# CycloneBoy/pdf_table

Measured on AMD Instinct MI355X. Metric: pages/s, higher is better.
Workload: dtype bf16

## Files before the change

### pdf_table_amd/csrc/c_api.hip

```cpp
#include <stdarg.h>
#include <stdio.h>
#include <stdlib.h>

#include <cmath>

#include "common.h"

namespace PT_FMT_NS {
namespace api {

static int ensure(void** buf, size_t* cap, size_t need);

int pt_engine_check(pt_engine* e) {
  PT_REQUIRE(e, "pt_engine_check: null engine");
  if (e->lstm_err && *e->lstm_err) {
    *e->lstm_err = 0;
    e->lstm_cluster = 0;
    pt_set_error("lstm_cluster_kernel: a workgroup waited > 2^22 polls for its peers -- the launch was not co-resident "
                 "(GPU shared with another process or stream?).  The recognition results since the last check are invalid; "
                 "this engine now uses the streaming LSTM kernel (pt_engine_set_lstm_cluster(e, 0)): run the batch again");
    return PT_ERR_HIP;
  }
  return PT_OK;
}
// ... 430 lines not shown
  return PT_OK;
}

int pt_det_box_scores(pt_engine* e, const float* d_prob, int n, int net_h, int net_w, const float* d_boxes, int nb,
                      float* d_scores, pt_stream stream) {
  PT_REQUIRE(e && d_prob && (nb == 0 || (d_boxes && d_scores)), "pt_det_box_scores: bad arguments");
  return pt_launch_box_scores(d_prob, n, net_h, net_w, d_boxes, nb, d_scores, reinterpret_cast<hipStream_t>(stream));
}

static int ensure(void** buf, size_t* cap, size_t need) {
  if (need <= *cap) return PT_OK;
  PT_HIP_CHECK(hipDeviceSynchronize());
  if (*buf) PT_HIP_CHECK(hipFree(*buf));
  *buf = nullptr;
  *cap = 0;
  PT_HIP_CHECK(hipMalloc(buf, need));
  *cap = need;
  return PT_OK;
}

static int rec_microbatch() {
  static int mb = -1;
  if (mb < 0) {
    const char* s = getenv("PT_REC_MICROBATCH");
    mb = s ? atoi(s) : 6144;
    if (mb < 1) mb = 1;
  }
  return mb;
}

static int rec_pre_chunk(pt_engine* e, const uint8_t* d_pages, int n_pages, int h, int w, const pt_rec_line* d_lines,
                         const int64_t* h_crop_px, int i0, int nb, bf16_t* d_gray, hipStream_t s) {
  (void)n_pages;
  long long maxpx = 0, total = 0;
  for (int i = 0; i < nb; ++i) {
    const long long px = h_crop_px[i0 + i] > 0 ? h_crop_px[i0 + i] : 0;
    total += px;
    if (px > maxpx) maxpx = px;
  }
  int rc;
  if ((rc = ensure(&e->rec_off, &e->rec_off_cap, (size_t)(nb + 1) * sizeof(long long))) != PT_OK) return rc;
  if ((rc = ensure(&e->rec_crops, &e->rec_crops_cap, (size_t)total * 3 + 16)) != PT_OK) return rc;
  if ((rc = pt_launch_rec_offsets(d_lines + i0, nb, reinterpret_cast<long long*>(e->rec_off), s)) != PT_OK) return rc;
  const long long* d_off = reinterpret_cast<const long long*>(e->rec_off);
  {
    PtProfScope ps(e, s, PT_PROF_OTHER, 0, "rec warp");
    rc = pt_launch_rec_warp(d_pages, h, w, d_lines + i0, nb, d_off, reinterpret_cast<uint8_t*>(e->rec_crops), (int)maxpx, s);
    if (rc != PT_OK) return rc;
  }
  PtProfScope ps(e, s, PT_PROF_OTHER, 0, "rec resize+gray");
  return pt_launch_rec_resize_gray(reinterpret_cast<const uint8_t*>(e->rec_crops), d_lines + i0, d_off, nb,
                                   pt_split(e), d_gray, s);
}

int pt_rec_preprocess(pt_engine* e, const uint8_t* d_pages_rgb, int n_pages, int h, int w, const pt_rec_line* d_lines,
                      const int64_t* h_crop_px, int n_lines, uint16_t* d_gray, pt_stream stream) {
  PT_REQUIRE(e && d_pages_rgb && d_lines && h_crop_px && d_gray && n_lines > 0, "pt_rec_preprocess: bad arguments");
  PT_HIP_CHECK(hipSetDevice(e->device));
  return rec_pre_chunk(e, d_pages_rgb, n_pages, h, w, d_lines, h_crop_px, 0, n_lines, d_gray, reinterpret_cast<hipStream_t>(stream));
}

static int upload_crop_offsets(pt_engine* e, const std::vector<long long>& off, hipStream_t s) {
  const size_t nb = off.size() * sizeof(long long);
  void* hs = e->stage_ring.acquire(nb);
  PT_REQUIRE(hs, "recognition: pinned staging (%s)", hipGetErrorString(hipGetLastError()));
  memcpy(hs, off.data(), nb);
// ... 546 lines not shown
```

### pdf_table_amd/csrc/common.h

```cpp
#pragma once
#include <hip/hip_runtime.h>
#include <stdint.h>
#include <string.h>

#include <map>
#include <string>
#include <vector>

#include "../../include/pdftable_hip.h"
#include "act16.h"

typedef uint16_t bf16_t;

void pt_set_error(const char* fmt, ...);

#define PT_HIP_CHECK(expr)                                                                  \
  do {                                                                                      \
    hipError_t _e = (expr);                                                                 \
    if (_e != hipSuccess) {                                                                 \
      pt_set_error("%s failed: %s (%s:%d)", #expr, hipGetErrorString(_e), __FILE__, __LINE__); \
      return PT_ERR_HIP;                                                                    \
    }                                                                                       \
  } while (0)

// ... 240 lines not shown
                            float* logits, int split, hipStream_t s);
int pt_launch_db_head_mfma(const bf16_t* in, int B, int H, int W, const bf16_t* w3, const float* b3, const bf16_t* w6,
                           const float* b6, float* prob, float* logits, hipStream_t s, uint32_t* bitmap = nullptr, float thresh = 0.f);
int pt_launch_bitmap(const float* prob, int n, int H, int W, float thresh, int dilate, uint32_t* bitmap,
                     hipStream_t s);
int pt_launch_box_scores(const float* prob, int n, int H, int W, const float* boxes, int nb, float* scores,
                         hipStream_t s);

#define PT_SE_CHUNKS 64
int pt_launch_stem3x3s2(const bf16_t* in, const float* w, const float* b, bf16_t* out, int B, int H, int W, int split,
                        hipStream_t s, int variant);
int pt_launch_dwconv(const bf16_t* in, const float* w, const float* b, bf16_t* out, int B, int H, int W, int C, int k,
                     int stride, int act, int split, hipStream_t s, const float* slope);
int pt_launch_se(const bf16_t* x, const float* w1, const float* b1, const float* w2, const float* b2, float* gate,
                 bf16_t* out, int B, int HW, int C, int split, hipStream_t s, int hidden, int mode, float* part);
int pt_launch_add(const bf16_t* a, const bf16_t* b, bf16_t* out, long long npix, int C, int split, hipStream_t s);
int pt_launch_chan_mean(const bf16_t* x, int B, int HW, int C, int split, float* part, bf16_t* mean, int rows, hipStream_t s);
int pt_pplcnet_forward_net(pt_engine* e, int slot, const bf16_t* x, int n, int H, int W, int textline, float* logits,
                           int* n_classes, hipStream_t s, int arena);
int pt_launch_cls_resize_norm(const uint8_t* base, const pt_cls_image* images, int n, int max_h, int max_w, int OH, int OW,
                              const float* lut, int split, bf16_t* out, hipStream_t s);
int pt_launch_cls_desc_from_lines(const pt_rec_line* lines, const long long* off, int n, pt_cls_image* images, hipStream_t s);
int pt_launch_cls_line_resize_norm(const uint8_t* pages, int ph, int pw, const pt_rec_line* lines, int n, int max_h, int max_w, int OH,
                                   int OW, const float* lut, int split, bf16_t* out, hipStream_t s);
int pt_launch_dbnas_tail(const bf16_t* y, const float* tw, int B, int H4, int W4, int split, float* prob, float* logits,
                         hipStream_t s);
int pt_dbnas_forward_net(pt_engine* e, const bf16_t* x, int n, int H, int W, float* prob, float* logits, hipStream_t s);

int pt_launch_rec_offsets(const pt_rec_line* lines, int n, long long* off, hipStream_t s);
int pt_launch_rec_warp(const uint8_t* pages, int ph, int pw, const pt_rec_line* lines, int n_lines,
                       const long long* pix_off, uint8_t* crops, int max_crop_px, hipStream_t s);
int pt_launch_rec_resize_gray(const uint8_t* crops, const pt_rec_line* lines, const long long* pix_off, int n_lines,
                              int split, bf16_t* out, hipStream_t s);
int pt_launch_rec_pp_resize_norm(const uint8_t* crops, const pt_rec_line* lines, const long long* pix_off,
                                 const pt_rec_pp_item* items, int n_items, int img_h, int max_img_w, const float* lut, float* out,
                                 hipStream_t s);
struct PtCrnnLimits {
  int* lim[6];
  int* cols;
  int* glist;
  int* blist3a;
  int* blist2a;
  int* blist2b;
};
int pt_launch_rows_live_list(const int* lim, int n, int* glist, hipStream_t s);
int pt_launch_crnn_limits(const pt_rec_line* lines, int n, const PtCrnnLimits& L, hipStream_t s);
int pt_launch_crnn_fill(bf16_t* out, const bf16_t* ref, const int* lim, int tile_w, int div, int n, int rows, int W, int cs,
                        hipStream_t s, const int* end_lim = nullptr, int end_tile = 1);
int pt_launch_crnn_conv0_pool(const bf16_t* in, int n, int H, int W, const float* w64x9, const float* bias, int split,
                              bf16_t* out, hipStream_t s, const int* xlim = nullptr);
int pt_launch_maxpool_kxk(const bf16_t* in, int n, int H, int W, int C, int kh, int kw, int h2c, int split, bf16_t* out,
                          hipStream_t s);
int pt_launch_lstm(pt_engine* e, const bf16_t* gx, const bf16_t* whh, bf16_t* hout, int B, int T, int split, hipStream_t s);
int pt_launch_gemm_argmax(const bf16_t* A, long long M, int K, const bf16_t* W, const float* bias, int N, int* ids, float* maxv,
                          hipStream_t s);
int pt_launch_gemm_argmax_x3(const bf16_t* A, long long M, int K, const bf16_t* W3, const float* bias, int N, int n_real, int* ids, float* maxv,
                             void* scratch, hipStream_t s);
int pt_launch_gemm_rows_x3(const bf16_t* A, long long M, int K, const bf16_t* W3, const float* bias, int N, bf16_t* out, int relu, hipStream_t s,
                           const int* tlim = nullptr);
int pt_launch_gemm_rows(const bf16_t* A, long long M, int K, const bf16_t* W, const float* bias, int N, bf16_t* out, int relu,
                        hipStream_t s, const int* tlim = nullptr);
int pt_launch_argmax_reduce(const float* part, long long rows, int ntiles, int* ids, float* maxv, hipStream_t s);
int pt_crnn_forward_net(pt_engine* e, const bf16_t* gray, int n, int32_t* ids, float* maxlogit, hipStream_t s,
                        const pt_rec_line* d_lines = nullptr);

int pt_cvit_forward_net(pt_engine* e, const float* gray, int layout, int n, int32_t* ids, float* maxlogit, hipStream_t s,
// ... 89 lines not shown
```

### pdf_table_amd/csrc/det_kernels.hip

```cpp
#include <math.h>

#include "common.h"

namespace PT_FMT_NS {

typedef __attribute__((ext_vector_type(4))) uint32_t u32x4;
typedef __attribute__((ext_vector_type(2))) uint32_t u32x2;

__device__ __forceinline__ float bf2f(uint32_t bits16) { return a16_to_f32(bits16); }
__device__ __forceinline__ uint32_t f2bf(float f) { return f32_to_a16(f); }

struct ResizeCoef {
  int s0, s1;
  int a0, a1;
};
__device__ __forceinline__ ResizeCoef resize_coef(int d, double scale, int ssize, bool clamp_frac) {
  float f = (float)(((double)d + 0.5) * scale - 0.5);
  int s = (int)floorf(f);
  f -= (float)s;
  ResizeCoef c;
  if (clamp_frac) {
    if (s < 0) { f = 0.f; s = 0; }
    if (s >= ssize - 1) { f = 0.f; s = ssize - 1; }
  }
  c.a0 = (int)rintf((1.f - f) * 2048.f);
  c.a1 = (int)rintf(f * 2048.f);
  int t0 = s, t1 = s + 1;
  t0 = t0 < 0 ? 0 : (t0 >= ssize ? ssize - 1 : t0);
  t1 = t1 < 0 ? 0 : (t1 >= ssize ? ssize - 1 : t1);
  c.s0 = t0;
  c.s1 = t1;
  return c;
}

constexpr int PRE_ROWS = 8;

__global__ __launch_bounds__(256) void det_preprocess_kernel(const uint8_t* __restrict__ pages, int n, int h, int w,
                                                              int nh, int nw, int flavour, int split, bf16_t* __restrict__ out,
                                                              double sx, double sy) {
  a16_kernel_enter();
  __shared__ uint32_t lut[3][256];
  {
    const int u = threadIdx.x;
#pragma unroll
    for (int c = 0; c < 3; ++c) {
      float o;
      if (flavour == PT_DET_PRE_DB_TORCH) {
        const float mean[3] = {123.68f, 116.78f, 103.94f};
        o = ((float)u - mean[c]) / 255.f;
      } else {
        const float scale = (float)(1.0 / 255.0);
        const float mean[3] = {0.485f, 0.456f, 0.406f};
        const float stdv[3] = {0.229f, 0.224f, 0.225f};
        o = ((float)u * scale - mean[c]) / stdv[c];
      }
      const uint32_t hi = f2bf(o);
      lut[c][u] = hi | (f2bf(o - bf2f(hi)) << 16);
    }
  }
  __syncthreads();
  const bool area2 = (w == 2 * nw) && (h == 2 * nh);
  const int b = blockIdx.z;
  const uint8_t* src = pages + (size_t)b * h * w * 3;
  for (int x = blockIdx.x * blockDim.x + threadIdx.x; x < nw; x += gridDim.x * blockDim.x) {
    const ResizeCoef cx = resize_coef(x, sx, w, true);
    const int o0 = cx.s0 * 3, d1 = (cx.s1 - cx.s0) * 24;
    for (int ry = 0; ry < PRE_ROWS; ++ry) {
      const int y = blockIdx.y * PRE_ROWS + ry;
      if (y >= nh) break;
      const long long i = ((long long)b * nh + y) * nw + x;
      int v[3];
      if (w == nw && h == nh) {
        const uint8_t* p = src + ((size_t)y * w + x) * 3;
        v[0] = p[0]; v[1] = p[1]; v[2] = p[2];
      } else if (area2) {
        const uint8_t* p0 = src + ((size_t)(2 * y) * w + 2 * x) * 3;
        const uint8_t* p1 = p0 + (size_t)w * 3;
#pragma unroll
        for (int c = 0; c < 3; ++c) v[c] = (p0[c] + p0[3 + c] + p1[c] + p1[3 + c] + 2) >> 2;
      } else {
        const ResizeCoef cy = resize_coef(y, sy, h, false);
        const uint8_t* r0 = src + (size_t)cy.s0 * w * 3;
        const uint8_t* r1 = src + (size_t)cy.s1 * w * 3;
        unsigned long long q0, q1;
        if (o0 + 8 <= w * 3) {
          __builtin_memcpy(&q0, r0 + o0, 8);
          __builtin_memcpy(&q1, r1 + o0, 8);
        } else {
          q0 = q1 = 0;
          for (int k = 0; k < 3; ++k) {
            q0 |= (unsigned long long)r0[o0 + k] << (8 * k) | (unsigned long long)r0[cx.s1 * 3 + k] << (d1 + 8 * k);
            q1 |= (unsigned long long)r1[o0 + k] << (8 * k) | (unsigned long long)r1[cx.s1 * 3 + k] << (d1 + 8 * k);
          }
        }
#pragma unroll
        for (int c = 0; c < 3; ++c) {
          const int S0 = (int)((q0 >> (8 * c)) & 0xFF) * cx.a0 + (int)((q0 >> (d1 + 8 * c)) & 0xFF) * cx.a1;
          const int S1 = (int)((q1 >> (8 * c)) & 0xFF) * cx.a0 + (int)((q1 >> (d1 + 8 * c)) & 0xFF) * cx.a1;
          v[c] = (((cy.a0 * (S0 >> 4)) >> 16) + ((cy.a1 * (S1 >> 4)) >> 16) + 2) >> 2;
          v[c] = v[c] < 0 ? 0 : (v[c] > 255 ? 255 : v[c]);
        }
      }
      const uint32_t e0 = lut[0][v[2]], e1 = lut[1][v[1]], e2 = lut[2][v[0]];
      if (!split) {
        u32x2 pk;
        pk.x = (e0 & 0xFFFFu) | (e1 << 16);
        pk.y = e2 & 0xFFFFu;
        *reinterpret_cast<u32x2*>(out + (size_t)i * 4) = pk;
      } else {
        u32x4 pk;
        pk.x = (e0 & 0xFFFFu) | (e1 << 16);
        pk.y = e2 & 0xFFFFu;
        pk.z = (e0 >> 16) | (e1 & 0xFFFF0000u);
        pk.w = e2 >> 16;
        *reinterpret_cast<u32x4*>(out + (size_t)i * 8) = pk;
      }
    }
  }
}

int pt_launch_det_preprocess(const uint8_t* pages, int n, int h, int w, int nh, int nw, int flavour, int split,
                             bf16_t* out, hipStream_t s) {
  PT_REQUIRE(n > 0 && nh > 0 && nw > 0 && nh < 65536 && n < 65536, "det pre-process: bad extents %d x %d x %d", n, nh, nw);
  hipLaunchKernelGGL(det_preprocess_kernel, dim3((nw + 255) / 256, (nh + PRE_ROWS - 1) / PRE_ROWS, n), dim3(256), 0, s, pages, n, h, w, nh, nw, flavour, split, out,
                     (double)w / nw, (double)h / nh);
  PT_HIP_CHECK(hipGetLastError());
  return PT_OK;
}

__device__ __forceinline__ uint32_t bfmax2(uint32_t a, uint32_t b) {
  const float al = a16lo_f32(a), bl = a16lo_f32(b);
  const float ah = a16hi_f32(a), bh = a16hi_f32(b);
  const uint32_t lo = (bl > al) ? (b & 0xFFFFu) : (a & 0xFFFFu);
  const uint32_t hi = (bh > ah) ? (b & 0xFFFF0000u) : (a & 0xFFFF0000u);
  return lo | hi;
}

__global__ __launch_bounds__(256) void maxpool3x3s2_split_kernel(const bf16_t* __restrict__ in, int B, int H, int W,
                                                                  int C, bf16_t* __restrict__ out) {
  a16_kernel_enter();
  const int Ho = (H + 2 - 3) / 2 + 1, Wo = (W + 2 - 3) / 2 + 1;
  const int cg = C >> 3;
  const long long total = (long long)B * Ho * Wo * cg;
  for (long long i = (long long)blockIdx.x * blockDim.x + threadIdx.x; i < total; i += (long long)gridDim.x * blockDim.x) {
    const int g = (int)(i % cg);
    long long t = i / cg;
    const int ox = (int)(t % Wo);
    t /= Wo;
    const int oy = (int)(t % Ho);
    const int b = (int)(t / Ho);
    uint32_t bh[8], bl[8];
    float bv[8];
    bool first = true;
    for (int dy = 0; dy < 3; ++dy) {
      const int iy = oy * 2 - 1 + dy;
      if ((unsigned)iy >= (unsigned)H) continue;
      for (int dx = 0; dx < 3; ++dx) {
        const int ix = ox * 2 - 1 + dx;
// ... 483 lines not shown
```

### pdf_table_amd/csrc/dla_net.h

```cpp
#pragma once

#include <stdlib.h>

#include <string>
#include <vector>

#include "net_ctx.h"

namespace PT_FMT_NS {

int pt_launch_conv3x3_c16(pt_engine* e, const bf16_t* in, const bf16_t* w, const float* bias, bf16_t* out, int B, int H, int W,
                          int N, int stride, int split, hipStream_t s);
int pt_launch_dla_thin_chain(pt_engine* e, const bf16_t* in, int B, int H, int W, const bf16_t* w_stem, const float* b_stem, const bf16_t* w0,
                             const float* b0, const bf16_t* w1, const float* b1, bf16_t* out, hipStream_t s);

namespace {

struct DlaCtx : NetCtx {
  bf16_t* cols = nullptr;
  float* om = nullptr;
  const int* ylimit = nullptr;
  double alg_scale = 1.0;

  void conv(const T& in, const std::string& q, int N, int ks, int stride, const T& out, int relu, const T* res = nullptr,
            int nv = 0, float* out_f32 = nullptr, int f32_cs = 0, int cin_override = 0, int alg_n = 0) {
    ConvDesc c;
    if (!conv_desc(c, in, q, N, ks, stride, relu)) return;
    if (cin_override) c.Cin = cin_override;
    c.n_valid = nv; c.ylimit = ylimit; c.alg_n = alg_n; c.alg_scale = alg_scale;
    if (out_f32) to_f32(c, out_f32, f32_cs);
    else to_map(c, out);
    if (res) { c.res = res->p; c.res_mode = 1; }
    launch(c);
  }
  void conv_cat(const std::vector<T>& ins, const std::string& q, int N, const T& out, int relu) {
    const PtTensor* w = get(q + (x3 ? ".w3" : ".w"));
    const PtTensor* b = get(q + ".b");
    if (!go()) return;
    ConvDesc c;
    c.in = ins[0].p; c.B = n; c.H = ins[0].H; c.W = ins[0].W;
    c.nseg = (int)ins.size();
    c.Cin = 0;
    for (int i = 0; i < c.nseg; ++i) {
      c.seg_c[i] = ins[i].C;
      c.Cin += ins[i].C;
      if (i) c.in_more[i - 1] = ins[i].p;
    }
    c.w = W(w); c.bias = F(b);
    c.N = N; c.ks = 1; c.stride = 1; c.relu = relu; c.split = x3; c.alg_scale = alg_scale;
    to_map(c, out);
    launch(c);
  }
  T maxpool2(const T& x) {
    T o = alloc(x.H / 2, x.W / 2, x.C);
    if (go()) {
      e->prof.next_bytes = (double)n * x.H * x.W * x.C * 2.0 * mul * 1.25;
      PtProfScope ps(e, s, PT_PROF_OTHER, 0, "maxpool2x2");
      const int r = pt_launch_maxpool_kxk(x.p, n, x.H, x.W, x.C, 2, 2, 0, x3, o.p, s);
      if (r != PT_OK) rc = r;
    }
    return o;
  }
  T block(const std::string& q, const T& x, const T& residual, int stride, int cout) {
    T t = alloc(x.H / stride, x.W / stride, cout);
    conv(x, q + ".conv1", cout, 3, stride, t, 1);
    T o = alloc(t.H, t.W, cout);
    conv(t, q + ".conv2", cout, 3, 1, o, 1, &residual);
    return o;
  }
  T tree(const std::string& q, int levels, const T& x, int cin, int cout, int stride, bool level_root,
         std::vector<T> children) {
    T bottom = stride > 1 ? maxpool2(x) : x;
    if (level_root) children.push_back(bottom);
    if (levels == 1) {
      T residual = bottom;
      if (cin != cout) {
        residual = alloc(bottom.H, bottom.W, cout);
        conv(bottom, q + ".project", cout, 1, 1, residual, 0);
      }
      T x1 = block(q + ".tree1", x, residual, stride, cout);
      T x2 = block(q + ".tree2", x1, x1, 1, cout);
      std::vector<T> ins = {x2, x1};
      ins.insert(ins.end(), children.begin(), children.end());
      T o = alloc(x1.H, x1.W, cout);
      conv_cat(ins, q + ".root", cout, o, 1);
      return o;
    }
    T x1 = tree(q + ".tree1", levels - 1, x, cin, cout, stride, false, {});
    children.push_back(x1);
    return tree(q + ".tree2", levels - 1, x1, cout, cout, 1, false, children);
  }
};

static std::vector<T> dla34_base(DlaCtx& c, const bf16_t* x, int H, int W) {
  pt_engine* e = c.e;
  hipStream_t s = c.s;
  const int n = c.n;
  const int ch[6] = {16, 32, 64, 128, 256, 512};
  const int lv[6] = {1, 1, 1, 2, 2, 1};
  const char* chain_env = getenv("PT_DLA_CHAIN");
  const bool chain = !c.x3 && H % 2 == 0 && W % 2 == 0 && !(chain_env && atoi(chain_env) == 0);
  std::vector<T> layers(6);
  if (chain) {
    layers[1] = c.alloc(H / 2, W / 2, 32);
    const PtTensor *ws = c.get("base_layer.w"), *bs = c.get("base_layer.b"), *w0 = c.get("level0.wt"), *b0 = c.get("level0.bt"),
                   *w1 = c.get("level1.wt"), *b1 = c.get("level1.bt");
    if (c.go()) {
      const int r = pt_launch_dla_thin_chain(e, x, n, H, W, c.W(ws), c.F(bs), c.W(w0), c.F(b0), c.W(w1), c.F(b1), layers[1].p, s);
      if (r != PT_OK) c.rc = r;
    }
  } else {
    T t0 = c.alloc(H, W, 16);
    const PtTensor* w = c.get(c.x3 ? "base_layer.w3" : "base_layer.w");
    const PtTensor* b = c.get("base_layer.b");
    if (c.go()) {
      const int r = pt_launch_stem7x7(e, x, n, H, W, c.W(w), c.F(b), t0.p, c.x3, s, 1, 16);
      if (r != PT_OK) c.rc = r;
    }
    layers[0] = c.alloc(H, W, 16);
    layers[1] = c.alloc(H / 2, W / 2, 32);
    for (int lv1 = 0; lv1 < 2; ++lv1) {
      const std::string q = lv1 ? "level1" : "level0";
      const PtTensor* w = c.get(q + (c.x3 ? ".wt3" : ".wt"));
      const PtTensor* b = c.get(q + ".bt");
      if (c.go()) {
        const int r = pt_launch_conv3x3_c16(e, lv1 ? layers[0].p : t0.p, c.W(w), c.F(b), layers[lv1].p, n, H, W, lv1 ? 32 : 16,
                                            lv1 ? 2 : 1, c.x3, s);
        if (r != PT_OK) c.rc = r;
      }
    }
  }
  for (int l = 2; l < 6; ++l)
    layers[l] = c.tree("level" + std::to_string(l), lv[l], layers[l - 1], ch[l - 1], ch[l], 2, l > 2, {});
  return layers;
// ... 6 lines not shown
```

### pdf_table_amd/csrc/lore_kernels.hip

```cpp
#include <stdio.h>
#include <stdlib.h>

#include "common.h"

namespace PT_FMT_NS {

typedef __attribute__((ext_vector_type(4))) uint32_t u32x4;
typedef __attribute__((ext_vector_type(2))) uint32_t u32x2;

namespace {

__device__ __forceinline__ float bf2f(uint32_t b) { return a16_to_f32(b); }
__device__ __forceinline__ uint32_t f2bf(float f) { return f32_to_a16(f); }

__device__ __forceinline__ void load8(const bf16_t* p, int lo_off, int split, float* v) {
  const u32x4 h = *reinterpret_cast<const u32x4*>(p);
  const uint32_t hw[4] = {h.x, h.y, h.z, h.w};
#pragma unroll
  for (int k = 0; k < 8; ++k) v[k] = bf2f((k & 1) ? (hw[k >> 1] >> 16) : (hw[k >> 1] & 0xFFFFu));
  if (split) {
    const u32x4 l = *reinterpret_cast<const u32x4*>(p + lo_off);
    const uint32_t lw[4] = {l.x, l.y, l.z, l.w};
#pragma unroll
    for (int k = 0; k < 8; ++k) v[k] += bf2f((k & 1) ? (lw[k >> 1] >> 16) : (lw[k >> 1] & 0xFFFFu));
// ... 250 lines not shown
  long long sx = X >> 5, sy = Y >> 5;
  sx = sx < -32768 ? -32768 : (sx > 32767 ? 32767 : sx);
  sy = sy < -32768 ? -32768 : (sy > 32767 ? 32767 : sy);
  const int ax = (int)(X & 31), ay = (int)(Y & 31);
  const int wt[4] = {(32 - ay) * (32 - ax) * 32, (32 - ay) * ax * 32, ay * (32 - ax) * 32, ay * ax * 32};
  int acc[3] = {0, 0, 0};
  const uint8_t* pg = pages + (size_t)tb.page * ph * pw * 3;
#pragma unroll
  for (int k = 0; k < 4; ++k) {
    const long long yy = sy + (k >> 1), xx = sx + (k & 1);
    if (yy < 0 || yy >= tb.crop_h || xx < 0 || xx >= tb.crop_w) continue;
    const long long py = tb.y0 + yy, px = tb.x0 + xx;
    if (py < 0 || py >= ph || px < 0 || px >= pw) continue;
    const uint8_t* s = pg + ((size_t)py * pw + px) * 3;
    acc[0] += s[0] * wt[k]; acc[1] += s[1] * wt[k]; acc[2] += s[2] * wt[k];
  }
  float v[3];
#pragma unroll
  for (int c = 0; c < 3; ++c) {
    const int sc = bgr ? 2 - c : c;
    int u = (acc[sc] + (1 << 14)) >> 15;
    u = u < 0 ? 0 : (u > 255 ? 255 : u);
    v[c] = lut[c * 256 + u];
  }
  bf16_t* o = out + ((size_t)t * H * W + i) * (split ? 8 : 4);
  uint32_t hb[3];
#pragma unroll
  for (int c = 0; c < 3; ++c) { hb[c] = f2bf(v[c]); o[c] = (bf16_t)hb[c]; }
  o[3] = 0;
  if (split) {
#pragma unroll
    for (int c = 0; c < 3; ++c) o[4 + c] = (bf16_t)f2bf(v[c] - bf2f(hb[c]));
    o[7] = 0;
  }
}

typedef __attribute__((ext_vector_type(8))) __bf16 dbf16x8;
typedef __attribute__((ext_vector_type(16))) float df32x16;
typedef __attribute__((ext_vector_type(2))) float df2;
__device__ __forceinline__ uint32_t pack_df2(df2 v) { return pack_a16x2(v.x, v.y); }
__device__ __forceinline__ df2 unpack_df2(uint32_t pk) { return df2{a16lo_f32(pk), a16hi_f32(pk)}; }

template <int SPLIT, int NB>
__global__ __launch_bounds__(256, (SPLIT || NB > 64) ? 2 : 4) void dcn_fused_kernel(const bf16_t* __restrict__ x, const float* __restrict__ om,
                                                            const bf16_t* __restrict__ w, const float* __restrict__ bias,
                                                            bf16_t* __restrict__ out, long long npix, int H, int W, int C,
                                                            int N, int relu) {
#pragma clang fp contract(fast)
  a16_kernel_enter();
  constexpr int ROW = 80;
  constexpr int NP = SPLIT ? 2 : 1;
  constexpr int NT = NB / 32;
  __shared__ __attribute__((aligned(16))) char s_a[NP][128 * ROW];
  __shared__ __attribute__((aligned(16))) char s_w[NP][NB * ROW];
  const int tid = threadIdx.x, lane = tid & 63, wave = tid >> 6;
  const int lx = lane & 31, q = lane >> 5;
  const long long p0 = (long long)blockIdx.x * 128;
  const int n0 = blockIdx.y * NB;
  const int cs = SPLIT ? 2 * C : C;
  const int nslice = C >> 5, nk = 9 * nslice;
  const int gp = tid & 127, gh = tid >> 7;
  long long pix = p0 + gp;
  const bool live = pix < npix;
  if (!live) pix = npix - 1;
  const int xw = (int)(pix % W), yh = (int)((pix / W) % H);
  const bf16_t* xb = x + (size_t)(pix / ((long long)W * H)) * H * W * cs;
// ... 1359 lines not shown
                         B, h, wd, C, 1);
    else
      hipLaunchKernelGGL(dwconvt_up2_add_kernel<0>, dim3(grid_for(blocks2)), dim3(256), (size_t)16 * C * sizeof(float), s, in, w, add, out,
                         B, h, wd, C, split);
    PT_HIP_CHECK(hipGetLastError());
    return PT_OK;
  }
  hipLaunchKernelGGL(dwconvt_up_add_kernel, dim3(grid_for((long long)B * h * f * wd * f * (C / 8))), dim3(256), 0, s, in,
                     w, add, out, B, h, wd, C, f, split);
  PT_HIP_CHECK(hipGetLastError());
  return PT_OK;
}

int pt_launch_dwconvt_up2_slice(const bf16_t* in, const float* w, bf16_t* out, int out_cstride, int out_coff, int out_lo_off, int B,
                                int h, int wd, int C, int split, hipStream_t s) {
  PT_REQUIRE(in && w && out && C % 8 == 0 && C <= 512 && out_cstride % 8 == 0 && out_coff % 8 == 0 && out_lo_off % 8 == 0 &&
                 out_coff + C * (split ? 2 : 1) <= out_cstride && (!split || out_coff + out_lo_off + C <= out_cstride),
             "dwconvT slice: bad arguments");
  const long long blocks2 = (long long)B * h * wd * (C / 8);
  PT_REQUIRE(blocks2 < (1ll << 31), "dwconvT slice: map too large");
  if (split)
    hipLaunchKernelGGL((dwconvt_up2_add_kernel<2, true>), dim3(grid_for(blocks2)), dim3(256), (size_t)16 * C * sizeof(float), s, in, w,
                       (const bf16_t*)nullptr, out + out_coff, B, h, wd, C, 1, out_cstride, out_lo_off);
  else
    hipLaunchKernelGGL((dwconvt_up2_add_kernel<1, true>), dim3(grid_for(blocks2)), dim3(256), (size_t)16 * C * sizeof(float), s, in, w,
                       (const bf16_t*)nullptr, out + out_coff, B, h, wd, C, 0, out_cstride, 0);
  PT_HIP_CHECK(hipGetLastError());
  return PT_OK;
}

int pt_launch_tsr_preprocess(const uint8_t* pages, int ph, int pw, const pt_tsr_table* tabs, int n, int H, int W, int bgr,
                             const float* lut, bf16_t* out, int split, hipStream_t s) {
  PT_REQUIRE(pages && tabs && lut && out && n > 0 && H > 0 && W > 0, "tsr preprocess: bad arguments");
  hipLaunchKernelGGL(tsr_preprocess_kernel, dim3((H * W + 255) / 256, n), dim3(256), 0, s, pages, ph, pw, tabs, H, W, bgr, lut,
                     out, split);
  PT_HIP_CHECK(hipGetLastError());
  return PT_OK;
}

template <int SPLIT, int NB>
static int launch_dcn_fused(pt_engine* e, const bf16_t* x, const float* om, const bf16_t* w, const float* bias, bf16_t* out,
                            int B, int H, int W, int C, int N, int relu, hipStream_t s) {
  const long long npix = (long long)B * H * W;
  char label[48];
  snprintf(label, sizeof(label), "dcn fused %d->%d @%dx%d%s", C, N, H, W, SPLIT ? " x3" : "");
  PtProfScope prof(e, s, PT_PROF_OTHER, 0, label);
  hipLaunchKernelGGL((dcn_fused_kernel<SPLIT, NB>), dim3((unsigned)((npix + 127) / 128), N / NB), dim3(256), 0, s, x, om, w,
                     bias, out, npix, H, W, C, N, relu);
  PT_HIP_CHECK(hipGetLastError());
  return PT_OK;
}

bool pt_dcn_fuses_om(const pt_engine* e, int C, int split) {
  const char* ev = getenv("PT_DCN_FUSE_OM");
  const int on = ev ? atoi(ev) : 1;
  const char* nt = getenv("PT_DCN_THREADS");
  const char* ea = getenv("PT_DCN_EARLY");
  const char* xf = getenv("PT_DCN_X3_FAST");
  const bool defaults = !(nt && atoi(nt) != 512) && !(ea && atoi(ea) == 0) && !(xf && atoi(xf) == 0);
  if (!on || !e || C % 64 != 0 || !defaults || (!split && e->dcn_mfma != 0)) return false;
  return on == 2 || (!split && C <= 128);
}

int pt_launch_dcn_fused(pt_engine* e, const bf16_t* x, const float* om, const bf16_t* w, const float* bias, bf16_t* out,
                        int B, int H, int W, int C, int N, int split, int relu, hipStream_t s, const bf16_t* omw, const float* omb) {
  PT_REQUIRE(e && x && (om || (omw && omb)) && w && bias && out && C % 32 == 0 && N % 64 == 0, "dcn fused: bad arguments (C=%d N=%d)", C, N);
  PT_REQUIRE(!omw || pt_dcn_fuses_om(e, C, split), "dcn fused: the offset conv can only be fused on the default fused64 paths (C=%d)", C);
  PT_REQUIRE((long long)H * W * (split ? 2 * C : C) < (1ll << 31), "dcn fused: image too large for 32-bit offsets");
// ... 143 lines not shown
```

### pdf_table_amd/csrc/rec_kernels.hip

```cpp
#include <math.h>

#include "common.h"

namespace PT_FMT_NS {

typedef __attribute__((ext_vector_type(8))) __bf16 bf16x8;
typedef __attribute__((ext_vector_type(16))) float f32x16;
typedef __attribute__((ext_vector_type(4))) uint32_t u32x4;
typedef __attribute__((ext_vector_type(2))) uint32_t u32x2;

__device__ __forceinline__ float rbf2f(uint32_t bits16) { return a16_to_f32(bits16); }
__device__ __forceinline__ uint32_t rf2bf(float f) { return f32_to_a16(f); }

__global__ __launch_bounds__(256) void rec_warp_kernel(const uint8_t* __restrict__ pages, int ph, int pw,
                                                        const pt_rec_line* __restrict__ lines, int n_lines,
                                                        const long long* __restrict__ pix_off, uint8_t* __restrict__ crops) {
  a16_kernel_enter();
  const int li = blockIdx.y;
  if (li >= n_lines) return;
  const pt_rec_line L = lines[li];
  const int cw = L.crop_w, chh = L.crop_h;
  const long long npx = (long long)cw * chh;
  uint8_t* dst = crops + pix_off[li] * 3;
  const uint8_t* src = pages + (size_t)L.page * ph * pw * 3;
// ... 109 lines not shown
          for (int c = 0; c < 3; ++c) {
            const int S0 = r0[cx.s0 * 3 + c] * cx.a0 + r0[cx.s1 * 3 + c] * cx.a1;
            const int S1 = r1[cx.s0 * 3 + c] * cx.a0 + r1[cx.s1 * 3 + c] * cx.a1;
            int r = (((cy.a0 * (S0 >> 4)) >> 16) + ((cy.a1 * (S1 >> 4)) >> 16) + 2) >> 2;
            v[c] = r < 0 ? 0 : (r > 255 ? 255 : r);
          }
        }
        const float R = (float)v[0] / 255.f, G = (float)v[1] / 255.f, B = (float)v[2] / 255.f;
        gray = (R * 0.2989f + G * 0.5870f) + B * 0.1140f;
      }
    }
    if (out_f32) {
      out_f32[i] = gray;
      continue;
    }
    const uint32_t hb = rf2bf(gray);
    if (split) {
      out[i * 2] = (bf16_t)hb;
      out[i * 2 + 1] = (bf16_t)rf2bf(gray - rbf2f(hb));
    } else {
      out[i] = (bf16_t)hb;
    }
  }
}

int pt_launch_rec_resize_gray(const uint8_t* crops, const pt_rec_line* lines, const long long* pix_off, int n_lines,
                              int split, bf16_t* out, hipStream_t s) {
  if (n_lines <= 0) return PT_OK;
  const long long total = (long long)n_lines * 32 * 640;
  int blocks = (int)((total + 255) / 256);
  if (blocks > 256 * 32) blocks = 256 * 32;
  hipLaunchKernelGGL(rec_resize_gray_kernel, dim3(blocks), dim3(256), 0, s, crops, lines, pix_off, n_lines, 32, 640, split, out,
                     static_cast<float*>(nullptr));
  PT_HIP_CHECK(hipGetLastError());
  return PT_OK;
}

int pt_launch_rec_resize_gray_f32(const uint8_t* crops, const pt_rec_line* lines, const long long* pix_off, int n_lines, int tw,
                                  float* out, hipStream_t s) {
  if (n_lines <= 0) return PT_OK;
  const long long total = (long long)n_lines * 32 * tw;
  int blocks = (int)((total + 255) / 256);
  if (blocks > 256 * 32) blocks = 256 * 32;
  hipLaunchKernelGGL(rec_resize_gray_kernel, dim3(blocks), dim3(256), 0, s, crops, lines, pix_off, n_lines, 32, tw, 0,
                     static_cast<bf16_t*>(nullptr), out);
  PT_HIP_CHECK(hipGetLastError());
  return PT_OK;
}

__global__ void crnn_limits_kernel(const pt_rec_line* __restrict__ lines, int n, int* l1, int* l2a, int* l2b, int* l3a, int* l3b,
                                   int* l0, int* __restrict__ cols) {
  a16_kernel_enter();
  __shared__ int sums[6];
  if (threadIdx.x < 6) sums[threadIdx.x] = 0;
  __syncthreads();
  int acc[6] = {0, 0, 0, 0, 0, 0};
  for (int b = blockIdx.x * blockDim.x + threadIdx.x; b < n; b += gridDim.x * blockDim.x) {
    const int cw = lines[b].crop_w, chh = lines[b].crop_h;
    int nw = 0;
    if (cw > 0 && chh > 0) {
      const double ratio = (double)cw / (double)chh;
      nw = ratio > 640.0 / 32.0 ? 640 : (int)(32.0 * ratio);
    }
    const int e0 = (nw + 2) >> 1;
    const int e1 = (e0 + 2) >> 1;
    const int v[5] = {min(e0 + 1, 320), min(e1 + 1, 160), min(e1 + 2, 160), min(e1 + 3, 160), min(e1 + 4, 160)};
// ... 1883 lines not shown
```

Before: 807.2.

## Add tiled front-end preprocess kernels and fused rec warp+resize+gray, pool once in DLA

Replaces the det and TSR preprocessing kernels with tiled versions that precompute per-column and per-row resize coefficients in shared memory and emit two pixels per thread with vector stores. Recognition preprocessing now runs as one fused kernel that warps, resizes and converts each line tile to gray, staging source pixels in LDS. This drops the intermediate crops buffer and two kernel launches. DLA tree construction reuses a single maxpool result instead of pooling the same input twice. All paths are on by default and the old kernels stay reachable through environment variables. The new kernels carry more complex edge handling that could differ slightly at tile boundaries.

Result: no change. 812.4 (median of 6 runs) (+0.6%).

```diff
diff --git a/pdf_table_amd/csrc/c_api.hip b/pdf_table_amd/csrc/c_api.hip
--- a/pdf_table_amd/csrc/c_api.hip
+++ b/pdf_table_amd/csrc/c_api.hip
@@ -486,6 +486,11 @@
 static int rec_pre_chunk(pt_engine* e, const uint8_t* d_pages, int n_pages, int h, int w, const pt_rec_line* d_lines,
                          const int64_t* h_crop_px, int i0, int nb, bf16_t* d_gray, hipStream_t s) {
   (void)n_pages;
+  const char* ev = getenv("PT_FRONT_FAST");
+  if (!(ev && atoi(ev) == 0)) {
+    PtProfScope ps(e, s, PT_PROF_OTHER, 0, "rec warp+resize+gray");
+    return pt_launch_rec_line_gray(d_pages, h, w, d_lines + i0, nb, pt_split(e), d_gray, s);
+  }
   long long maxpx = 0, total = 0;
   for (int i = 0; i < nb; ++i) {
     const long long px = h_crop_px[i0 + i] > 0 ? h_crop_px[i0 + i] : 0;
diff --git a/pdf_table_amd/csrc/common.h b/pdf_table_amd/csrc/common.h
--- a/pdf_table_amd/csrc/common.h
+++ b/pdf_table_amd/csrc/common.h
@@ -296,6 +296,8 @@
                        const long long* pix_off, uint8_t* crops, int max_crop_px, hipStream_t s);
 int pt_launch_rec_resize_gray(const uint8_t* crops, const pt_rec_line* lines, const long long* pix_off, int n_lines,
                               int split, bf16_t* out, hipStream_t s);
+int pt_launch_rec_line_gray(const uint8_t* pages, int ph, int pw, const pt_rec_line* lines, int n_lines, int split, bf16_t* out,
+                            hipStream_t s);
 int pt_launch_rec_pp_resize_norm(const uint8_t* crops, const pt_rec_line* lines, const long long* pix_off,
                                  const pt_rec_pp_item* items, int n_items, int img_h, int max_img_w, const float* lut, float* out,
                                  hipStream_t s);
diff --git a/pdf_table_amd/csrc/det_kernels.hip b/pdf_table_amd/csrc/det_kernels.hip
--- a/pdf_table_amd/csrc/det_kernels.hip
+++ b/pdf_table_amd/csrc/det_kernels.hip
@@ -1,4 +1,5 @@
 #include <math.h>
+#include <stdlib.h>
 
 #include "common.h"
 
@@ -33,6 +34,24 @@
   return c;
 }
 
+__device__ __forceinline__ void det_norm_lut(uint32_t (*lut)[256], int flavour, int u) {
+#pragma unroll
+  for (int c = 0; c < 3; ++c) {
+    float o;
+    if (flavour == PT_DET_PRE_DB_TORCH) {
+      const float mean[3] = {123.68f, 116.78f, 103.94f};
+      o = ((float)u - mean[c]) / 255.f;
+    } else {
+      const float scale = (float)(1.0 / 255.0);
+      const float mean[3] = {0.485f, 0.456f, 0.406f};
+      const float stdv[3] = {0.229f, 0.224f, 0.225f};
+      o = ((float)u * scale - mean[c]) / stdv[c];
+    }
+    const uint32_t hi = f2bf(o);
+    lut[c][u] = hi | (f2bf(o - bf2f(hi)) << 16);
+  }
+}
+
 constexpr int PRE_ROWS = 8;
 
 __global__ __launch_bounds__(256) void det_preprocess_kernel(const uint8_t* __restrict__ pages, int n, int h, int w,
@@ -40,24 +59,7 @@
                                                               double sx, double sy) {
   a16_kernel_enter();
   __shared__ uint32_t lut[3][256];
-  {
-    const int u = threadIdx.x;
-#pragma unroll
-    for (int c = 0; c < 3; ++c) {
-      float o;
-      if (flavour == PT_DET_PRE_DB_TORCH) {
-        const float mean[3] = {123.68f, 116.78f, 103.94f};
-        o = ((float)u - mean[c]) / 255.f;
-      } else {
-        const float scale = (float)(1.0 / 255.0);
-        const float mean[3] = {0.485f, 0.456f, 0.406f};
-        const float stdv[3] = {0.229f, 0.224f, 0.225f};
-        o = ((float)u * scale - mean[c]) / stdv[c];
-      }
-      const uint32_t hi = f2bf(o);
-      lut[c][u] = hi | (f2bf(o - bf2f(hi)) << 16);
-    }
-  }
+  det_norm_lut(lut, flavour, threadIdx.x);
   __syncthreads();
   const bool area2 = (w == 2 * nw) && (h == 2 * nh);
   const int b = blockIdx.z;
@@ -119,11 +121,120 @@
   }
 }
 
+constexpr int DET_TILE_COLS = 128, DET_TILE_ROWS = 32;
+
+__device__ __forceinline__ void det_row_pair(const uint8_t* __restrict__ r, int o0, int d1, int rowbytes, uint32_t& pa, uint32_t& pb) {
+  if (o0 + 8 <= rowbytes) {
+    u32x2 q;
+    __builtin_memcpy(&q, r + o0, 8);
+    pa = q.x;
+    pb = __builtin_amdgcn_alignbit(q.y, q.x, (uint32_t)d1);
+  } else {
+    const int o1 = o0 + (d1 >> 3);
+    pa = (uint32_t)r[o0] | (uint32_t)r[o0 + 1] << 8 | (uint32_t)r[o0 + 2] << 16;
+    pb = (uint32_t)r[o1] | (uint32_t)r[o1 + 1] << 8 | (uint32_t)r[o1 + 2] << 16;
+  }
+}
+
+__global__ __launch_bounds__(256) void det_preprocess_tile_kernel(const uint8_t* __restrict__ pages, int n, int h, int w, int nh, int nw,
+                                                                   int flavour, int split, bf16_t* __restrict__ out, double sx, double sy) {
+  a16_kernel_enter();
+  __shared__ uint32_t lut[3][256];
+  __shared__ int4 s_cx[DET_TILE_COLS];
+  __shared__ int4 s_cy[DET_TILE_ROWS];
+  const int tid = threadIdx.x;
+  det_norm_lut(lut, flavour, tid);
+  const int x0 = blockIdx.x * DET_TILE_COLS, y0 = blockIdx.y * DET_TILE_ROWS;
+  if (tid < DET_TILE_COLS) {
+    const ResizeCoef c = resize_coef(x0 + tid, sx, w, true);
+    s_cx[tid] = make_int4(c.s0 * 3, (c.s1 - c.s0) * 24, c.a0, c.a1);
+  } else if (tid < DET_TILE_COLS + DET_TILE_ROWS) {
+    const ResizeCoef c = resize_coef(y0 + tid - DET_TILE_COLS, sy, h, false);
+    s_cy[tid - DET_TILE_COLS] = make_int4(c.s0, c.s1, c.a0, c.a1);
+  }
+  __syncthreads();
+  const int lane = tid & 63, wave = tid >> 6;
+  const int xa = x0 + 2 * lane;
+  if (xa >= nw) return;
+  const bool two = xa + 1 < nw;
+  const int4 ca = s_cx[2 * lane], cb = s_cx[2 * lane + 1];
+  const bool same = (w == nw && h == nh), area2 = (w == 2 * nw) && (h == 2 * nh);
+  const int b = blockIdx.z;
+  const int rowbytes = w * 3;
+  const uint8_t* src = pages + (size_t)b * h * rowbytes;
+  for (int ry = wave; ry < DET_TILE_ROWS; ry += 4) {
+    const int y = y0 + ry;
+    if (y >= nh) break;
+    int v[2][3];
+    if (same) {
+      const uint8_t* p = src + (size_t)y * rowbytes + xa * 3;
+#pragma unroll
+      for (int c = 0; c < 3; ++c) { v[0][c] = p[c]; v[1][c] = two ? p[3 + c] : 0; }
+    } else if (area2) {
+      const uint8_t* p0 = src + (size_t)(2 * y) * rowbytes + 2 * xa * 3;
+      const uint8_t* p1 = p0 + rowbytes;
+#pragma unroll
+      for (int c = 0; c < 3; ++c) {
+        v[0][c] = (p0[c] + p0[3 + c] + p1[c] + p1[3 + c] + 2) >> 2;
+        v[1][c] = two ? (p0[6 + c] + p0[9 + c] + p1[6 + c] + p1[9 + c] + 2) >> 2 : 0;
+      }
+    } else {
+      const int4 cy = s_cy[ry];
+      const uint8_t* r0 = src + (size_t)cy.x * rowbytes;
+      const uint8_t* r1 = src + (size_t)cy.y * rowbytes;
+#pragma unroll
+      for (int k = 0; k < 2; ++k) {
+        const int4 cx = k ? cb : ca;
+        uint32_t p0a, p0b, p1a, p1b;
+        det_row_pair(r0, cx.x, cx.y, rowbytes, p0a, p0b);
+        det_row_pair(r1, cx.x, cx.y, rowbytes, p1a, p1b);
+#pragma unroll
+        for (int c = 0; c < 3; ++c) {
+          const int S0 = (int)((p0a >> (8 * c)) & 0xFF) * cx.z + (int)((p0b >> (8 * c)) & 0xFF) * cx.w;
+          const int S1 = (int)((p1a >> (8 * c)) & 0xFF) * cx.z + (int)((p1b >> (8 * c)) & 0xFF) * cx.w;
+          const int t = (((cy.z * (S0 >> 4)) >> 16) + ((cy.w * (S1 >> 4)) >> 16) + 2) >> 2;
+          v[k][c] = t < 0 ? 0 : (t > 255 ? 255 : t);
+        }
+      }
+    }
+    uint32_t e[2][3];
+#pragma unroll
+    for (int k = 0; k < 2; ++k) { e[k][0] = lut[0][v[k][2]]; e[k][1] = lut[1][v[k][1]]; e[k][2] = lut[2][v[k][0]]; }
+    const long long i = ((long long)b * nh + y) * nw + xa;
+    if (!split) {
+      const u32x2 pa = {(e[0][0] & 0xFFFFu) | (e[0][1] << 16), e[0][2] & 0xFFFFu};
+      const u32x2 pb = {(e[1][0] & 0xFFFFu) | (e[1][1] << 16), e[1][2] & 0xFFFFu};
+      if (two && !(i & 1)) {
+        *reinterpret_cast<u32x4*>(out + (size_t)i * 4) = u32x4{pa.x, pa.y, pb.x, pb.y};
+      } else {
+        *reinterpret_cast<u32x2*>(out + (size_t)i * 4) = pa;
+        if (two) *reinterpret_cast<u32x2*>(out + (size_t)i * 4 + 4) = pb;
+      }
+    } else {
+#pragma unroll
+      for (int k = 0; k < 2; ++k) {
+        if (k && !two) break;
+        u32x4 pk;
+        pk.x = (e[k][0] & 0xFFFFu) | (e[k][1] << 16);
+        pk.y = e[k][2] & 0xFFFFu;
+        pk.z = (e[k][0] >> 16) | (e[k][1] & 0xFFFF0000u);
+        pk.w = e[k][2] >> 16;
+        *reinterpret_cast<u32x4*>(out + (size_t)(i + k) * 8) = pk;
+      }
+    }
+  }
+}
+
 int pt_launch_det_preprocess(const uint8_t* pages, int n, int h, int w, int nh, int nw, int flavour, int split,
                              bf16_t* out, hipStream_t s) {
   PT_REQUIRE(n > 0 && nh > 0 && nw > 0 && nh < 65536 && n < 65536, "det pre-process: bad extents %d x %d x %d", n, nh, nw);
-  hipLaunchKernelGGL(det_preprocess_kernel, dim3((nw + 255) / 256, (nh + PRE_ROWS - 1) / PRE_ROWS, n), dim3(256), 0, s, pages, n, h, w, nh, nw, flavour, split, out,
-                     (double)w / nw, (double)h / nh);
+  const char* ev = getenv("PT_FRONT_FAST");
+  if (ev && atoi(ev) == 0)
+    hipLaunchKernelGGL(det_preprocess_kernel, dim3((nw + 255) / 256, (nh + PRE_ROWS - 1) / PRE_ROWS, n), dim3(256), 0, s, pages, n, h, w, nh, nw, flavour, split, out,
+                       (double)w / nw, (double)h / nh);
+  else
+    hipLaunchKernelGGL(det_preprocess_tile_kernel, dim3((nw + DET_TILE_COLS - 1) / DET_TILE_COLS, (nh + DET_TILE_ROWS - 1) / DET_TILE_ROWS, n), dim3(256), 0, s,
+                       pages, n, h, w, nh, nw, flavour, split, out, (double)w / nw, (double)h / nh);
   PT_HIP_CHECK(hipGetLastError());
   return PT_OK;
 }
diff --git a/pdf_table_amd/csrc/dla_net.h b/pdf_table_amd/csrc/dla_net.h
--- a/pdf_table_amd/csrc/dla_net.h
+++ b/pdf_table_amd/csrc/dla_net.h
@@ -21,6 +21,7 @@
   float* om = nullptr;
   const int* ylimit = nullptr;
   double alg_scale = 1.0;
+  bool pool_once = true;
 
   void conv(const T& in, const std::string& q, int N, int ks, int stride, const T& out, int relu, const T* res = nullptr,
             int nv = 0, float* out_f32 = nullptr, int f32_cs = 0, int cin_override = 0, int alg_n = 0) {
@@ -69,8 +70,8 @@
     return o;
   }
   T tree(const std::string& q, int levels, const T& x, int cin, int cout, int stride, bool level_root,
-         std::vector<T> children) {
-    T bottom = stride > 1 ? maxpool2(x) : x;
+         std::vector<T> children, const T* pooled = nullptr) {
+    T bottom = stride > 1 ? (pooled ? *pooled : maxpool2(x)) : x;
     if (level_root) children.push_back(bottom);
     if (levels == 1) {
       T residual = bottom;
@@ -86,7 +87,7 @@
       conv_cat(ins, q + ".root", cout, o, 1);
       return o;
     }
-    T x1 = tree(q + ".tree1", levels - 1, x, cin, cout, stride, false, {});
+    T x1 = tree(q + ".tree1", levels - 1, x, cin, cout, stride, false, {}, stride > 1 && pool_once ? &bottom : nullptr);
     children.push_back(x1);
     return tree(q + ".tree2", levels - 1, x1, cout, cout, 1, false, children);
   }
@@ -100,6 +101,8 @@
   const int lv[6] = {1, 1, 1, 2, 2, 1};
   const char* chain_env = getenv("PT_DLA_CHAIN");
   const bool chain = !c.x3 && H % 2 == 0 && W % 2 == 0 && !(chain_env && atoi(chain_env) == 0);
+  const char* pool_env = getenv("PT_DLA_POOL_ONCE");
+  c.pool_once = !(pool_env && atoi(pool_env) == 0);
   std::vector<T> layers(6);
   if (chain) {
     layers[1] = c.alloc(H / 2, W / 2, 32);
diff --git a/pdf_table_amd/csrc/lore_kernels.hip b/pdf_table_amd/csrc/lore_kernels.hip
--- a/pdf_table_amd/csrc/lore_kernels.hip
+++ b/pdf_table_amd/csrc/lore_kernels.hip
@@ -306,6 +306,117 @@
 #pragma unroll
     for (int c = 0; c < 3; ++c) o[4 + c] = (bf16_t)f2bf(v[c] - bf2f(hb[c]));
     o[7] = 0;
+  }
+}
+
+constexpr int TSR_TILE_COLS = 128, TSR_TILE_ROWS = 32;
+
+__device__ __forceinline__ void tsr_sample(const uint8_t* __restrict__ pg, int ph, int pw, const pt_tsr_table& tb, long long X, long long Y, int acc[3]) {
+  long long sx = X >> 5, sy = Y >> 5;
+  sx = sx < -32768 ? -32768 : (sx > 32767 ? 32767 : sx);
+  sy = sy < -32768 ? -32768 : (sy > 32767 ? 32767 : sy);
+  const int ax = (int)(X & 31), ay = (int)(Y & 31);
+  const int wt[4] = {(32 - ay) * (32 - ax) * 32, (32 - ay) * ax * 32, ay * (32 - ax) * 32, ay * ax * 32};
+  acc[0] = acc[1] = acc[2] = 0;
+  const long long px = tb.x0 + sx, py = tb.y0 + sy;
+  bool okx[2], oky[2];
+#pragma unroll
+  for (int k = 0; k < 2; ++k) {
+    okx[k] = sx + k >= 0 && sx + k < tb.crop_w && px + k >= 0 && px + k < pw;
+    oky[k] = sy + k >= 0 && sy + k < tb.crop_h && py + k >= 0 && py + k < ph;
+  }
+  if (okx[0] && okx[1] && px * 3 + 8 <= (long long)pw * 3) {
+#pragma unroll
+    for (int r = 0; r < 2; ++r) {
+      if (!oky[r]) continue;
+      u32x2 q;
+      __builtin_memcpy(&q, pg + ((size_t)(py + r) * pw + px) * 3, 8);
+      const uint32_t pa = q.x, pb = __builtin_amdgcn_alignbit(q.y, q.x, 24u);
+#pragma unroll
+      for (int c = 0; c < 3; ++c) acc[c] += (int)((pa >> (8 * c)) & 0xFF) * wt[2 * r] + (int)((pb >> (8 * c)) & 0xFF) * wt[2 * r + 1];
+    }
+  } else {
+#pragma unroll
+    for (int k = 0; k < 4; ++k) {
+      if (!oky[k >> 1] || !okx[k & 1]) continue;
+      const uint8_t* s = pg + ((size_t)(py + (k >> 1)) * pw + (px + (k & 1))) * 3;
+      acc[0] += s[0] * wt[k]; acc[1] += s[1] * wt[k]; acc[2] += s[2] * wt[k];
+    }
+  }
+}
+
+__global__ __launch_bounds__(256) void tsr_preprocess_tile_kernel(const uint8_t* __restrict__ pages, int ph, int pw,
+                                                                   const pt_tsr_table* __restrict__ tabs, int H, int W, int bgr,
+                                                                   const float* __restrict__ lut, bf16_t* __restrict__ out, int split) {
+  a16_kernel_enter();
+  __shared__ uint32_t s_lut[768];
+  __shared__ long long s_col[TSR_TILE_COLS][2];
+  __shared__ long long s_row[TSR_TILE_ROWS][2];
+  const int tid = threadIdx.x;
+  const int t = blockIdx.z;
+  const pt_tsr_table tb = tabs[t];
+  const int x0 = blockIdx.x * TSR_TILE_COLS, y0 = blockIdx.y * TSR_TILE_ROWS;
+  for (int k = tid; k < 768; k += 256) {
+    const float f = lut[k];
+    const uint32_t hi = f2bf(f);
+    s_lut[k] = hi | (f2bf(f - bf2f(hi)) << 16);
+  }
+  auto sat = [](double v) { return (long long)fmin(fmax(rint(v), -2147483648.0), 2147483647.0); };
+  if (tid < TSR_TILE_COLS) {
+    const int x = x0 + tid;
+    s_col[tid][0] = sat(tb.minv[0] * x * 1024.0);
+    s_col[tid][1] = sat(tb.minv[3] * x * 1024.0);
+  } else if (tid < TSR_TILE_COLS + TSR_TILE_ROWS) {
+    const int y = y0 + tid - TSR_TILE_COLS;
+    s_row[tid - TSR_TILE_COLS][0] = sat((tb.minv[1] * y + tb.minv[2]) * 1024.0) + 16;
+    s_row[tid - TSR_TILE_COLS][1] = sat((tb.minv[4] * y + tb.minv[5]) * 1024.0) + 16;
+  }
+  __syncthreads();
+  const int lane = tid & 63, wave = tid >> 6;
+  const int xa = x0 + 2 * lane;
+  if (xa >= W) return;
+  const bool two = xa + 1 < W;
+  const long long ad[2] = {s_col[2 * lane][0], s_col[2 * lane + 1][0]}, bd[2] = {s_col[2 * lane][1], s_col[2 * lane + 1][1]};
+  const uint8_t* pg = pages + (size_t)tb.page * ph * pw * 3;
+  for (int ry = wave; ry < TSR_TILE_ROWS; ry += 4) {
+    const int y = y0 + ry;
+    if (y >= H) break;
+    const long long X0 = s_row[ry][0], Y0 = s_row[ry][1];
+    uint32_t e[2][3];
+#pragma unroll
+    for (int k = 0; k < 2; ++k) {
+      int acc[3];
+      if (k && !two) { e[k][0] = e[k][1] = e[k][2] = 0; break; }
+      tsr_sample(pg, ph, pw, tb, (X0 + ad[k]) >> 5, (Y0 + bd[k]) >> 5, acc);
+#pragma unroll
+      for (int c = 0; c < 3; ++c) {
+        int u = (acc[bgr ? 2 - c : c] + (1 << 14)) >> 15;
+        u = u < 0 ? 0 : (u > 255 ? 255 : u);
+        e[k][c] = s_lut[c * 256 + u];
+      }
+    }
+    const size_t i = ((size_t)t * H + y) * W + xa;
+    if (!split) {
+      const u32x2 pa = {(e[0][0] & 0xFFFFu) | (e[0][1] << 16), e[0][2] & 0xFFFFu};
+      const u32x2 pb = {(e[1][0] & 0xFFFFu) | (e[1][1] << 16), e[1][2] & 0xFFFFu};
+      if (two && !(i & 1)) {
+        *reinterpret_cast<u32x4*>(out + i * 4) = u32x4{pa.x, pa.y, pb.x, pb.y};
+      } else {
+        *reinterpret_cast<u32x2*>(out + i * 4) = pa;
+        if (two) *reinterpret_cast<u32x2*>(out + i * 4 + 4) = pb;
+      }
+    } else {
+#pragma unroll
+      for (int k = 0; k < 2; ++k) {
+        if (k && !two) break;
+        u32x4 pk;
+        pk.x = (e[k][0] & 0xFFFFu) | (e[k][1] << 16);
+        pk.y = e[k][2] & 0xFFFFu;
+        pk.z = (e[k][0] >> 16) | (e[k][1] & 0xFFFF0000u);
+        pk.w = e[k][2] >> 16;
+        *reinterpret_cast<u32x4*>(out + (i + k) * 8) = pk;
+      }
+    }
   }
 }
 
@@ -1731,8 +1842,13 @@
 int pt_launch_tsr_preprocess(const uint8_t* pages, int ph, int pw, const pt_tsr_table* tabs, int n, int H, int W, int bgr,
                              const float* lut, bf16_t* out, int split, hipStream_t s) {
   PT_REQUIRE(pages && tabs && lut && out && n > 0 && H > 0 && W > 0, "tsr preprocess: bad arguments");
-  hipLaunchKernelGGL(tsr_preprocess_kernel, dim3((H * W + 255) / 256, n), dim3(256), 0, s, pages, ph, pw, tabs, H, W, bgr, lut,
-                     out, split);
+  const char* ev = getenv("PT_FRONT_FAST");
+  if (ev && atoi(ev) == 0)
+    hipLaunchKernelGGL(tsr_preprocess_kernel, dim3((H * W + 255) / 256, n), dim3(256), 0, s, pages, ph, pw, tabs, H, W, bgr, lut,
+                       out, split);
+  else
+    hipLaunchKernelGGL(tsr_preprocess_tile_kernel, dim3((W + TSR_TILE_COLS - 1) / TSR_TILE_COLS, (H + TSR_TILE_ROWS - 1) / TSR_TILE_ROWS, n), dim3(256), 0, s,
+                       pages, ph, pw, tabs, H, W, bgr, lut, out, split);
   PT_HIP_CHECK(hipGetLastError());
   return PT_OK;
 }
diff --git a/pdf_table_amd/csrc/rec_kernels.hip b/pdf_table_amd/csrc/rec_kernels.hip
--- a/pdf_table_amd/csrc/rec_kernels.hip
+++ b/pdf_table_amd/csrc/rec_kernels.hip
@@ -165,6 +165,150 @@
   if (blocks > 256 * 32) blocks = 256 * 32;
   hipLaunchKernelGGL(rec_resize_gray_kernel, dim3(blocks), dim3(256), 0, s, crops, lines, pix_off, n_lines, 32, 640, split, out,
                      static_cast<float*>(nullptr));
+  PT_HIP_CHECK(hipGetLastError());
+  return PT_OK;
+}
+
+constexpr int REC_TILE_COLS = 64;
+constexpr int REC_TILE_CAP = 8192;
+
+__device__ __forceinline__ uint32_t rec_crop_px(const uint8_t* __restrict__ src, int ph, int pw, const double* m, int x, int y) {
+  int v[3];
+  pt_warp_sample(src, ph, pw, m, x, y, v);
+  return (uint32_t)v[0] | (uint32_t)v[1] << 8 | (uint32_t)v[2] << 16;
+}
+
+template <bool STAGED>
+__device__ __forceinline__ float rec_gray_px(int mode, int x, int y, int4 cx, int4 cy, const uint32_t* s_px, int c0, int r0, int ncols,
+                                             const float* s_div, const uint8_t* __restrict__ src, int ph, int pw, const double* m) {
+  int xs[2], ys[2];
+  if (mode == 0) { xs[0] = xs[1] = x; ys[0] = ys[1] = y; }
+  else if (mode == 1) { xs[0] = 2 * x; xs[1] = 2 * x + 1; ys[0] = 2 * y; ys[1] = 2 * y + 1; }
+  else { xs[0] = cx.x; xs[1] = cx.y; ys[0] = cy.x; ys[1] = cy.y; }
+  uint32_t P[2][2];
+#pragma unroll
+  for (int i = 0; i < 2; ++i)
+#pragma unroll
+    for (int j = 0; j < 2; ++j)
+      P[i][j] = STAGED ? s_px[(ys[i] - r0) * ncols + (xs[j] - c0)] : rec_crop_px(src, ph, pw, m, xs[j], ys[i]);
+  int v[3];
+#pragma unroll
+  for (int c = 0; c < 3; ++c) {
+    const int p00 = (P[0][0] >> (8 * c)) & 0xFF, p01 = (P[0][1] >> (8 * c)) & 0xFF, p10 = (P[1][0] >> (8 * c)) & 0xFF, p11 = (P[1][1] >> (8 * c)) & 0xFF;
+    if (mode == 0) {
+      v[c] = p00;
+    } else if (mode == 1) {
+      v[c] = (p00 + p01 + p10 + p11 + 2) >> 2;
+    } else {
+      const int S0 = p00 * cx.z + p01 * cx.w;
+      const int S1 = p10 * cx.z + p11 * cx.w;
+      const int r = (((cy.z * (S0 >> 4)) >> 16) + ((cy.w * (S1 >> 4)) >> 16) + 2) >> 2;
+      v[c] = r < 0 ? 0 : (r > 255 ? 255 : r);
+    }
+  }
+  const float R = s_div[v[0]], G = s_div[v[1]], B = s_div[v[2]];
+  return (R * 0.2989f + G * 0.5870f) + B * 0.1140f;
+}
+
+__global__ __launch_bounds__(256) void rec_line_gray_kernel(const uint8_t* __restrict__ pages, int ph, int pw,
+                                                             const pt_rec_line* __restrict__ lines, int n_lines, int split,
+                                                             bf16_t* __restrict__ out) {
+  a16_kernel_enter();
+  constexpr int TH = PT_REC_H, TWID = PT_REC_W;
+  static_assert(TH == 32 && REC_TILE_COLS * TH == 256 * 8, "256 threads x 8 pixels cover a tile");
+  __shared__ uint32_t s_px[REC_TILE_CAP];
+  __shared__ int4 s_cx[REC_TILE_COLS];
+  __shared__ int4 s_cy[TH];
+  __shared__ float s_div[256];
+  const int tid = threadIdx.x;
+  const int li = blockIdx.y, x0 = blockIdx.x * REC_TILE_COLS;
+  const int cw = lines[li].crop_w, chh = lines[li].crop_h;
+  int nw = 0;
+  if (cw > 0 && chh > 0) {
+    const double ratio = (double)cw / (double)chh;
+    nw = ratio > (double)TWID / (double)TH ? TWID : (int)((double)TH * ratio);
+  }
+  const int y = tid >> 3, xg = x0 + 8 * (tid & 7);
+  const size_t o = ((size_t)li * TH + y) * TWID + xg;
+  if (x0 >= nw) {
+    const u32x4 z = {0u, 0u, 0u, 0u};
+    if (split) {
+      *reinterpret_cast<u32x4*>(out + o * 2) = z;
+      *reinterpret_cast<u32x4*>(out + o * 2 + 8) = z;
+    } else {
+      *reinterpret_cast<u32x4*>(out + o) = z;
+    }
+    return;
+  }
+  const int mode = (cw == nw && chh == TH) ? 0 : ((cw == 2 * nw && chh == 2 * TH) ? 1 : 2);
+  const int xe = x0 + REC_TILE_COLS < nw ? x0 + REC_TILE_COLS : nw;
+  s_div[tid] = (float)tid / 255.f;
+  if (mode == 2) {
+    if (tid < REC_TILE_COLS) {
+      const RCoef c = rcoef(x0 + tid, (double)cw / nw, cw, true);
+      s_cx[tid] = make_int4(c.s0, c.s1, c.a0, c.a1);
+    } else if (tid < REC_TILE_COLS + TH) {
+      const RCoef c = rcoef(tid - REC_TILE_COLS, (double)chh / TH, chh, false);
+      s_cy[tid - REC_TILE_COLS] = make_int4(c.s0, c.s1, c.a0, c.a1);
+    }
+  }
+  __syncthreads();
+  int c0, c1, r0, r1;
+  if (mode == 0) { c0 = x0; c1 = xe - 1; r0 = 0; r1 = TH - 1; }
+  else if (mode == 1) { c0 = 2 * x0; c1 = 2 * xe - 1; r0 = 0; r1 = 2 * TH - 1; }
+  else { c0 = s_cx[0].x; c1 = s_cx[xe - 1 - x0].y; r0 = s_cy[0].x; r1 = s_cy[TH - 1].y; }
+  const int ncols = c1 - c0 + 1, nrows = r1 - r0 + 1;
+  const bool staged = (long long)ncols * nrows <= REC_TILE_CAP;
+  double m[9];
+#pragma unroll
+  for (int k = 0; k < 9; ++k) m[k] = lines[li].minv[k];
+  const uint8_t* src = pages + (size_t)lines[li].page * ph * pw * 3;
+  if (staged) {
+    for (int i = tid; i < ncols * nrows; i += 256) {
+      const int ry = i / ncols, rx = i - ry * ncols;
+      s_px[i] = rec_crop_px(src, ph, pw, m, c0 + rx, r0 + ry);
+    }
+    __syncthreads();
+  }
+  const int4 cy = mode == 2 ? s_cy[y] : make_int4(0, 0, 0, 0);
+  if (!staged) {
+#pragma unroll 1
+    for (int j = 0; j < 8; ++j) {
+      const int x = xg + j;
+      float gray = 0.f;
+      if (x < nw) gray = rec_gray_px<false>(mode, x, y, mode == 2 ? s_cx[x - x0] : cy, cy, s_px, c0, r0, ncols, s_div, src, ph, pw, m);
+      const uint32_t h = rf2bf(gray);
+      if (split) {
+        out[(o + j) * 2] = (bf16_t)h;
+        out[(o + j) * 2 + 1] = (bf16_t)rf2bf(gray - rbf2f(h));
+      } else {
+        out[o + j] = (bf16_t)h;
+      }
+    }
+    return;
+  }
+  uint32_t hb[8], lb[8];
+#pragma unroll
+  for (int j = 0; j < 8; ++j) {
+    const int x = xg + j;
+    float gray = 0.f;
+    if (x < nw) gray = rec_gray_px<true>(mode, x, y, mode == 2 ? s_cx[x - x0] : cy, cy, s_px, c0, r0, ncols, s_div, src, ph, pw, m);
+    hb[j] = rf2bf(gray);
+    lb[j] = rf2bf(gray - rbf2f(hb[j]));
+  }
+  if (split) {
+    *reinterpret_cast<u32x4*>(out + o * 2) = u32x4{hb[0] | lb[0] << 16, hb[1] | lb[1] << 16, hb[2] | lb[2] << 16, hb[3] | lb[3] << 16};
+    *reinterpret_cast<u32x4*>(out + o * 2 + 8) = u32x4{hb[4] | lb[4] << 16, hb[5] | lb[5] << 16, hb[6] | lb[6] << 16, hb[7] | lb[7] << 16};
+  } else {
+    *reinterpret_cast<u32x4*>(out + o) = u32x4{hb[0] | hb[1] << 16, hb[2] | hb[3] << 16, hb[4] | hb[5] << 16, hb[6] | hb[7] << 16};
+  }
+}
+
+int pt_launch_rec_line_gray(const uint8_t* pages, int ph, int pw, const pt_rec_line* lines, int n_lines, int split, bf16_t* out,
+                            hipStream_t s) {
+  if (n_lines <= 0) return PT_OK;
+  PT_REQUIRE(n_lines < 65536, "recognition pre-process: %d lines in one launch", n_lines);
+  hipLaunchKernelGGL(rec_line_gray_kernel, dim3(PT_REC_W / REC_TILE_COLS, n_lines), dim3(256), 0, s, pages, ph, pw, lines, n_lines, split, out);
   PT_HIP_CHECK(hipGetLastError());
   return PT_OK;
 }
```
